# akanazawa/human_dynamics

Hardware: AMD Instinct MI355X
Metric: frames/sec/GPU (ResNet+temporal+SMPL, 224x224); SMPL verts max-abs-err (higher is better)
Workload: dtype f16x3

## Files before the change

human_dynamics_amd/csrc/stem.hip:

```cpp
#include <type_traits>
#include <utility>

#include "common.h"
#include "hmmr_hip.h"

namespace {
constexpr int IMG = 224, CONV = 112, POOL = 56, CO = 64;
constexpr int PT = 8;
constexpr int CT = 2 * PT + 1;
constexpr int IP = 2 * CT + 5;
constexpr int IPW = 40;
constexpr int NPIX = CT * CT;
constexpr int MT = (NPIX + 31) / 32;
constexpr int TAPK = 32;
constexpr int WK = 256;

template <typename T> struct StemLds {
    static constexpr int PXB = 4 * (int)sizeof(T);
    static constexpr int PATCH = IP * IPW * PXB;
    static constexpr int WROW = 7 * TAPK * (int)sizeof(T) + 16;
    static constexpr int WTS = CO * WROW;
    static constexpr int CST = MT * 32 * CO * (int)sizeof(T);
    static constexpr int TOTAL = PATCH + (WTS > CST ? WTS : CST);
};

template <typename T> struct StemFrag;
template <> struct StemFrag<float> { typedef f32x4 type; };
template <> struct StemFrag<bf16_t> { typedef bf16x8 type; };

__device__ __forceinline__ f32x16 stem_mma(const f32x4& a, const f32x4& b, f32x16 c) {
#pragma unroll
    for (int j = 0; j < 4; ++j) c = __builtin_amdgcn_mfma_f32_32x32x2f32(a[j], b[j], c, 0, 0, 0);
    return c;
}
__device__ __forceinline__ f32x16 stem_mma(const bf16x8& a, const bf16x8& b, f32x16 c) {
    return __builtin_amdgcn_mfma_f32_32x32x16_bf16(a, b, c, 0, 0, 0);
}

__device__ __forceinline__ void store_rgbx(float* o, float r, float g, float b) {
    *(f32x4*)o = f32x4{r, g, b, 0.f};
}
__device__ __forceinline__ void store_rgbx(bf16_t* o, float r, float g, float b) {
    typedef __attribute__((ext_vector_type(4))) __bf16 bf16x4;
    *(bf16x4*)o = bf16x4{(bf16_t)r, (bf16_t)g, (bf16_t)b, (bf16_t)0.f};
}

template <typename T>
__global__ __launch_bounds__(256) void stem_fused_kernel(const float* __restrict__ img, const T* __restrict__ wts,
                                                         const float* __restrict__ bias,
                                                         const float* __restrict__ pscale,
                                                         const float* __restrict__ pshift, T* __restrict__ out,
                                                         int n_real, const T* __restrict__ w1,
                                                         const float* __restrict__ s1, const float* __restrict__ b1,
                                                         T* __restrict__ out_h1) {
    typedef StemLds<T> LD;
    typedef typename StemFrag<T>::type frag_t;
    constexpr int CPT = (int)sizeof(T);
    extern __shared__ __attribute__((aligned(16))) char smem[];
    char* s_patch = smem;
    char* s_w = smem + LD::PATCH;
    T* s_c = (T*)(smem + LD::PATCH);

    const int tid = threadIdx.x, lane = tid & 63;
    const int wave = __builtin_amdgcn_readfirstlane(tid >> 6);
    const int ty = blockIdx.x / (POOL / PT), tx = blockIdx.x % (POOL / PT);
    const int n = blockIdx.y;
    const int cy0 = 2 * PT * ty, cx0 = 2 * PT * tx;
    const int iy0 = 2 * cy0 - 3, ix0 = 2 * cx0 - 3;

    const float* im = img + (long long)n * IMG * IMG * 3;
    for (int i = tid; i < IP * 11; i += 256) {
        const int py = i / 11, q = i - py * 11;
        const int gy = iy0 + py, gx = ix0 - 1 + 4 * q;
        float f[12];
#pragma unroll
        for (int e = 0; e < 12; ++e) f[e] = 0.f;
        if (n < n_real && (unsigned)gy < (unsigned)IMG && (unsigned)gx < (unsigned)IMG) {
            const f32x4* p = (const f32x4*)(im + (gy * IMG + gx) * 3);
            const f32x4 v0 = p[0], v1 = p[1], v2 = p[2];
#pragma unroll
            for (int e = 0; e < 4; ++e) { f[e] = v0[e]; f[4 + e] = v1[e]; f[8 + e] = v2[e]; }
        }
#pragma unroll
        for (int e = 0; e < 4; ++e) {
            const int px = 4 * q - 1 + e;
            if ((unsigned)px < (unsigned)IPW) {
                T* o = (T*)(s_patch + (py * IPW + px) * LD::PXB);
                store_rgbx(o, f[3 * e], f[3 * e + 1], f[3 * e + 2]);
            }
        }
    }
    constexpr int SLOTS_PER_ROW = 7 * TAPK * (int)sizeof(T) / 16;
    for (int i = tid; i < CO * SLOTS_PER_ROW; i += 256) {
        const int row = i / SLOTS_PER_ROW, sl = i - row * SLOTS_PER_ROW;
        *(u32x4*)(s_w + row * LD::WROW + sl * 16) = *(const u32x4*)((const char*)(wts + (long long)row * WK) + sl * 16);
    }
    __syncthreads();

    const int lr = lane & 31, lh = lane >> 5;
    constexpr int MPW = (MT + 3) / 4;
    f32x16 acc[MPW][2];
#pragma unroll
    for (int i = 0; i < MPW; ++i)
#pragma unroll
        for (int j = 0; j < 2; ++j)
#pragma unroll
            for (int r = 0; r < 16; ++r) acc[i][j][r] = 0.f;
    int abase[MPW];
#pragma unroll
    for (int i = 0; i < MPW; ++i) {
        int p = (wave + 4 * i) * 32 + lr;
        if (p >= NPIX) p = 0;
        const int cy = p / CT, cx = p - cy * CT;
        abase[i] = ((2 * cy) * IPW + 2 * cx) * LD::PXB + lh * 16;
    }
    const int bbase = lr * LD::WROW + lh * 16;
#pragma unroll 1
    for (int ky = 0; ky < 7; ++ky) {
#pragma unroll
        for (int c = 0; c < CPT; ++c) {
            const frag_t b0 = *(const frag_t*)(s_w + bbase + ky * TAPK * (int)sizeof(T) + c * 32);
            const frag_t b1 = *(const frag_t*)(s_w + bbase + 32 * LD::WROW + ky * TAPK * (int)sizeof(T) + c * 32);
#pragma unroll
            for (int i = 0; i < MPW; ++i) {
                if (wave + 4 * i < MT) {
                    const frag_t a = *(const frag_t*)(s_patch + abase[i] + ky * IPW * LD::PXB + c * 32);
                    acc[i][0] = stem_mma(a, b0, acc[i][0]);
                    acc[i][1] = stem_mma(a, b1, acc[i][1]);
                }
            }
        }
    }
    __syncthreads();

#pragma unroll
    for (int i = 0; i < MPW; ++i) {
        if (wave + 4 * i < MT) {
#pragma unroll
            for (int j = 0; j < 2; ++j) {
                const int ch = j * 32 + lr;
                const float bch = bias[ch];
#pragma unroll
                for (int r = 0; r < 16; ++r) {
                    const int p = (wave + 4 * i) * 32 + (r & 3) + 8 * (r >> 2) + 4 * lh;
                    s_c[p * CO + ch] = elem_traits<T>::from_f32(acc[i][j][r] + bch);
                }
            }
        }
    }
    __syncthreads();

    for (int it = tid; it < PT * PT * (CO / 8); it += 256) {
        const int v8 = it & 7, pp = it >> 3;
        const int py = pp / PT, px = pp - py * PT;
        float m[8];
#pragma unroll
        for (int j = 0; j < 8; ++j) m[j] = -3.0e38f;
#pragma unroll
        for (int dy = 0; dy < 3; ++dy) {
            if (cy0 + 2 * py + dy >= CONV) continue;
#pragma unroll
            for (int dx = 0; dx < 3; ++dx) {
                if (cx0 + 2 * px + dx >= CONV) continue;
                float v[8];
                load8(s_c + ((2 * py + dy) * CT + 2 * px + dx) * CO + v8 * 8, v);
#pragma unroll
                for (int j = 0; j < 8; ++j) m[j] = fmaxf(m[j], v[j]);
            }
        }
        float sc[8], sh[8];
        load8(pscale + v8 * 8, sc); load8(pshift + v8 * 8, sh);
#pragma unroll
        for (int j = 0; j < 8; ++j) m[j] = fmaxf(fmaf(m[j], sc[j], sh[j]), 0.f);
        store8(out + (((long long)n * POOL + PT * ty + py) * POOL + PT * tx + px) * CO + v8 * 8, m);
        if constexpr (sizeof(T) == 2) {
            if (out_h1) store8((T*)(s_patch + pp * 128 + ((v8 ^ ((pp >> 1) & 7)) << 4)), m);
        }
    }
    if constexpr (sizeof(T) == 2) {
        if (!out_h1) return;
        __syncthreads();
        const int lr = lane & 31, lh = lane >> 5, fsw = (lr >> 1) & 7;
        const int wn = wave >> 1, wm = wave & 1;
        f32x16 acc1;
#pragma unroll
        for (int r = 0; r < 16; ++r) acc1[r] = 0.f;
#pragma unroll
        for (int kc = 0; kc < 4; ++kc) {
            const bf16x8 a = *(const bf16x8*)(w1 + (long long)(wn * 32 + lr) * 64 + kc * 16 + lh * 8);
            const bf16x8 b = *(const bf16x8*)(s_patch + (wm * 32 + lr) * 128 + (((2 * kc + lh) ^ fsw) << 4));
            acc1 = __builtin_amdgcn_mfma_f32_32x32x16_bf16(a, b, acc1, 0, 0, 0);
        }
        char* s_o = smem + LD::PATCH;
#pragma unroll
        for (int g = 0; g < 4; ++g) {
            const int cl = wn * 32 + 8 * g + 4 * lh;
            const f32x4 s4 = *(const f32x4*)(s1 + cl), b4 = *(const f32x4*)(b1 + cl);
            typedef __attribute__((ext_vector_type(4))) __bf16 bf16x4;
            bf16x4 o;
#pragma unroll
            for (int j = 0; j < 4; ++j) o[j] = (bf16_t)fmaxf(fmaf(acc1[4 * g + j], s4[j], b4[j]), 0.f);
            *(bf16x4*)(s_o + (wm * 32 + lr) * 128 + (((cl >> 3) ^ fsw) << 4) + 8 * lh) = o;
        }
        __syncthreads();
        for (int it = tid; it < PT * PT * (CO / 8); it += 256) {
            const int ps = it & 7, pp = it >> 3, ls = ps ^ ((pp >> 1) & 7);
            const int py = pp / PT, px = pp - py * PT;
            *(u32x4*)(out_h1 + (((long long)n * POOL + PT * ty + py) * POOL + PT * tx + px) * CO + ls * 8) =
                *(const u32x4*)(s_o + pp * 128 + ps * 16);
        }
    }
}
}


namespace {
constexpr int X3_NT = 320, X3_CO = 32;
constexpr int X3_PLANE = IP * IPW * 8;
constexpr int X3_WROW = 7 * TAPK * 2 + 16;
constexpr int X3_WPLANE = X3_CO * X3_WROW;
constexpr int X3_STAGE = MT * 32 * X3_CO * 4;
constexpr int X3_PTILE = PT * PT * 128;
constexpr int X3_LDS0 = 2 * X3_PLANE + (2 * X3_WPLANE > X3_STAGE ? 2 * X3_WPLANE : X3_STAGE);
constexpr int X3_LDS = X3_LDS0 + X3_PTILE;
static_assert(2 * X3_PTILE <= 2 * X3_PLANE + X3_PTILE && 2 * X3_LDS <= 160 * 1024, "two workgroups per CU");

__global__ __launch_bounds__(X3_NT) void stem_fused_split_kernel(const float* __restrict__ img, const bsplit_t* __restrict__ wts,
                                                                 const float* __restrict__ wscale,
                                                                 const float* __restrict__ bias, const float* __restrict__ pscale,
                                                                 const float* __restrict__ pshift, bsplit_t* __restrict__ out,
                                                                 int n_real, const char* __restrict__ w1f, const float* __restrict__ s1,
                                                                 const float* __restrict__ b1, bsplit_t* __restrict__ out_h1) {
    extern __shared__ __attribute__((aligned(16))) char smem[];
    char* s_ph = smem;
    char* s_pl = smem + X3_PLANE;
    char* s_wh = smem + 2 * X3_PLANE;
    char* s_wl = s_wh + X3_WPLANE;
    float* s_c = (float*)(smem + 2 * X3_PLANE);

    const int tid = threadIdx.x, lane = tid & 63;
    const int wave = __builtin_amdgcn_readfirstlane(tid >> 6);
    const int ty = blockIdx.x / (POOL / PT), tx = blockIdx.x % (POOL / PT);
    const int n = blockIdx.y;
    const int cy0 = 2 * PT * ty, cx0 = 2 * PT * tx;
    const int iy0 = 2 * cy0 - 3, ix0 = 2 * cx0 - 3;

    const float* im = img + (long long)n * IMG * IMG * 3;
    float satin = 0.f;
    for (int i = tid; i < IP * 11; i += X3_NT) {
        const int py = i / 11, q = i - py * 11;
        const int gy = iy0 + py, gx = ix0 - 1 + 4 * q;
        float f[12];
#pragma unroll
        for (int e = 0; e < 12; ++e) f[e] = 0.f;
        if (n < n_real && (unsigned)gy < (unsigned)IMG && (unsigned)gx < (unsigned)IMG) {
            const f32x4* p = (const f32x4*)(im + (gy * IMG + gx) * 3);
            const f32x4 v0 = p[0], v1 = p[1], v2 = p[2];
#pragma unroll
            for (int e = 0; e < 4; ++e) { f[e] = v0[e]; f[4 + e] = v1[e]; f[8 + e] = v2[e]; }
#pragma unroll
            for (int e = 0; e < 12; e += 2) satin = sat_acc(satin, f[e], f[e + 1]);
        }
#pragma unroll
        for (int e = 0; e < 4; ++e) {
            const int px = 4 * q - 1 + e;
            if ((unsigned)px < (unsigned)IPW) {
                typedef __attribute__((ext_vector_type(4))) shalf_t shalf4;
                shalf4 h, l;
#pragma unroll
                for (int c = 0; c < 3; ++c) {
                    const float cv = split_clamp(f[3 * e + c]);
                    h[c] = (shalf_t)cv;
                    l[c] = (shalf_t)(cv - (float)h[c]);
                }
                h[3] = (shalf_t)0.f; l[3] = (shalf_t)0.f;
                *(shalf4*)(s_ph + (py * IPW + px) * 8) = h;
                *(shalf4*)(s_pl + (py * IPW + px) * 8) = l;
            }
        }
    }
    split_flag_max(satin);
#pragma unroll 1
    for (int ch0 = 0; ch0 < CO; ch0 += X3_CO) {
    if (ch0) __syncthreads();
    for (int i = tid; i < X3_CO * 28; i += X3_NT) {
        const int row = i / 28, g = i - row * 28;
        const u32x4* src = (const u32x4*)((const char*)wts + (long long)(ch0 + row) * (WK * 4) + g * 32);
        *(u32x4*)(s_wh + row * X3_WROW + g * 16) = src[0];
        *(u32x4*)(s_wl + row * X3_WROW + g * 16) = src[1];
    }
    __syncthreads();

    const int lr = lane & 31, lh = lane >> 5;
    constexpr int MPW = MT / 5;
    static_assert(MPW * 5 == MT, "10 row tiles over 5 waves");
    f32x16 acc[MPW];
#pragma unroll
    for (int i = 0; i < MPW; ++i)
#pragma unroll
        for (int r = 0; r < 16; ++r) acc[i][r] = 0.f;
    int abase[MPW];
#pragma unroll
    for (int i = 0; i < MPW; ++i) {
        int p = (wave + 5 * i) * 32 + lr;
        if (p >= NPIX) p = 0;
        const int cy = p / CT, cx = p - cy * CT;
        abase[i] = ((2 * cy) * IPW + 2 * cx) * 8 + lh * 16;
    }
    const int bbase = lr * X3_WROW + lh * 16;
    const unsigned lds0 = (unsigned)(unsigned long long)(__attribute__((address_space(3))) void*)smem;
    const unsigned aw = lds0 + 2 * X3_PLANE + bbase;
    unsigned ap[MPW];
#pragma unroll
    for (int i = 0; i < MPW; ++i) ap[i] = lds0 + abase[i];
    shalf8 fb[2][2], fa[2][MPW][2];
#define STEM_RD(dst, addr, OFF) asm volatile("ds_read_b128 %0, %1 offset:%2" : "=v"(dst) : "v"(addr), "n"(OFF))
    auto load_step = [&](auto s_c, int set) {
        constexpr int S = decltype(s_c)::value, KY = S >> 1, C = S & 1;
        shalf8& bh = fb[set][0];
        shalf8& bl = fb[set][1];
        STEM_RD(bh, aw, KY * 64 + C * 32);
        STEM_RD(bl, aw, X3_WPLANE + KY * 64 + C * 32);
#pragma unroll
        for (int i = 0; i < MPW; ++i) {
            shalf8& ah = fa[set][i][0];
            shalf8& al = fa[set][i][1];
            const unsigned ad = ap[i];
            STEM_RD(ah, ad, KY * IPW * 8 + C * 32);
            STEM_RD(al, ad, X3_PLANE + KY * IPW * 8 + C * 32);
        }
    };
    auto k_step = [&](auto s_c) {
        constexpr int S = decltype(s_c)::value, CUR = S & 1;
        if constexpr (S + 1 < 14) load_step(std::integral_constant<int, (S + 1 < 14 ? S + 1 : 13)>{}, CUR ^ 1);
#pragma unroll
        for (int i = 0; i < MPW; ++i) {
            acc[i] = mfma_split(fa[CUR][i][1], fb[CUR][0], acc[i]);
            acc[i] = mfma_split(fa[CUR][i][0], fb[CUR][1], acc[i]);
            acc[i] = mfma_split(fa[CUR][i][0], fb[CUR][0], acc[i]);
        }
        __builtin_amdgcn_sched_barrier(0);
        __builtin_amdgcn_s_waitcnt(63 | (7 << 4) | (0 << 8) | (3 << 14));
        __builtin_amdgcn_sched_barrier(0);
    };
    load_step(std::integral_constant<int, 0>{}, 0);
    __builtin_amdgcn_s_waitcnt(63 | (7 << 4) | (0 << 8) | (3 << 14));
    __builtin_amdgcn_sched_barrier(0);
    auto k_steps = [&](auto... S) { (k_step(S), ...); };
    k_steps(std::integral_constant<int, 0>{}, std::integral_constant<int, 1>{}, std::integral_constant<int, 2>{}, std::integral_constant<int, 3>{},
            std::integral_constant<int, 4>{}, std::integral_constant<int, 5>{}, std::integral_constant<int, 6>{}, std::integral_constant<int, 7>{},
            std::integral_constant<int, 8>{}, std::integral_constant<int, 9>{}, std::integral_constant<int, 10>{}, std::integral_constant<int, 11>{},
            std::integral_constant<int, 12>{}, std::integral_constant<int, 13>{});
#undef STEM_RD
    __syncthreads();

    {
        const float bch = bias[ch0 + lr];
        const float sch = wscale ? wscale[ch0 + lr] : 1.0f;
#pragma unroll
        for (int i = 0; i < MPW; ++i)
#pragma unroll
            for (int r = 0; r < 16; ++r) {
                const int p = (wave + 5 * i) * 32 + (r & 3) + 8 * (r >> 2) + 4 * lh;
                s_c[p * X3_CO + lr] = stored_value<bsplit_t>(fmaf(acc[i][r], sch, bch));
            }
    }
    __syncthreads();

    for (int it = tid; it < PT * PT * (X3_CO / 8); it += X3_NT) {
        const int v8 = it & 3, pp = it >> 2;
        const int py = pp / PT, px = pp - py * PT;
        float m[8];
#pragma unroll
        for (int j = 0; j < 8; ++j) m[j] = -3.0e38f;
#pragma unroll
        for (int dy = 0; dy < 3; ++dy) {
            if (cy0 + 2 * py + dy >= CONV) continue;
#pragma unroll
            for (int dx = 0; dx < 3; ++dx) {
                if (cx0 + 2 * px + dx >= CONV) continue;
                float v[8];
                load8(s_c + ((2 * py + dy) * CT + 2 * px + dx) * X3_CO + v8 * 8, v);
#pragma unroll
                for (int j = 0; j < 8; ++j) m[j] = fmaxf(m[j], v[j]);
            }
        }
        float sc[8], sh[8];
        load8(pscale + ch0 + v8 * 8, sc); load8(pshift + ch0 + v8 * 8, sh);
#pragma unroll
        for (int j = 0; j < 8; ++j) m[j] = fmaxf(fmaf(m[j], sc[j], sh[j]), 0.f);
        bsplit_t* o = out + (((long long)n * POOL + PT * ty + py) * POOL + PT * tx + px) * CO + ch0 + v8 * 8;
        store8(o, m);
        if (w1f) {
            shalf8 hi, lo;
#pragma unroll
            for (int j = 0; j < 8; ++j) {
                const float cv = split_clamp(m[j]);
                hi[j] = (shalf_t)cv;
                lo[j] = (shalf_t)(cv - (float)hi[j]);
            }
            char* pt = (ch0 ? smem : smem + X3_LDS0) + pp * 128 + ((v8 ^ (pp & 3)) << 5);
            *(shalf8*)pt = hi;
            *(shalf8*)(pt + 16) = lo;
        }
    }
    }
    if (!w1f) return;
    __syncthreads();
    if (wave < 4) {
        const int lr = lane & 31, lh = lane >> 5;
        const int wn = wave >> 1, wm = wave & 1;
        const int p = wm * 32 + lr;
        f32x16 acc1;
#pragma unroll
        for (int r = 0; r < 16; ++r) acc1[r] = 0.f;
#pragma unroll
        for (int kc = 0; kc < 4; ++kc) {
            const shalf8* wp = (const shalf8*)(w1f + ((long long)((wn * 4 + kc) * 64 + lane)) * 32);
            wfrag wf; wf.hi = wp[0]; wf.lo = wp[1];
            const int g = (2 * kc + lh) & 3;
            const char* pt = (kc >= 2 ? smem : smem + X3_LDS0) + p * 128 + ((g ^ (p & 3)) << 5);
            acc1 = mma3(wf, *(const shalf8*)pt, *(const shalf8*)(pt + 16), acc1);
        }
        const int py = p >> 3, px = p & 7;
        bsplit_t* o = out_h1 + (((long long)n * POOL + PT * ty + py) * POOL + PT * tx + px) * CO;
        float satmax = 0.f;
#pragma unroll
        for (int g = 0; g < 4; ++g) {
            const int ch = wn * 32 + 8 * g + 4 * lh;
            const f32x4 s4 = *(const f32x4*)(s1 + ch), b4 = *(const f32x4*)(b1 + ch);
            float v[4];
#pragma unroll
            for (int e = 0; e < 4; ++e) v[e] = fmaf(acc1[4 * g + e], s4[e], b4[e]);
            unsigned h2[2], l2[2];
            split4_mix(v, 0.f, h2, l2, satmax);
            char* og = (char*)o + (wn * 4 + g) * 32 + 8 * lh;
            *(unsigned long long*)og = (unsigned long long)h2[0] | ((unsigned long long)h2[1] << 32);
            *(unsigned long long*)(og + 16) = (unsigned long long)l2[0] | ((unsigned long long)l2[1] << 32);
        }
        split_flag_max(satmax);
    }
}
}

int hmmr_stem_fused(const float* images, int n_real, int n, const void* wts, const float* wscale, const float* bias,
                    const float* pscale, const float* pshift, void* out, int dtype, hipStream_t s,
                    const void* w1, const float* s1, const float* b1, void* out_h1) {
    if (dtype == HMMR_F16X3) {
        auto kern = stem_fused_split_kernel;
        static DeviceOnce oncex3;
        if (const unsigned long long bit = oncex3.due()) {
            HMMR_CHECK_HIP(hipFuncSetAttribute((const void*)kern, hipFuncAttributeMaxDynamicSharedMemorySize, X3_LDS));
            oncex3.mark(bit);
        }
        hipLaunchKernelGGL(kern, dim3((POOL / PT) * (POOL / PT), n), dim3(X3_NT), X3_LDS, s, images,
                           (const bsplit_t*)wts, wscale, bias, pscale, pshift, (bsplit_t*)out, n_real, (const char*)w1, s1, b1,
                           (bsplit_t*)out_h1);
    } else if (dtype == HMMR_BF16) {
        auto kern = stem_fused_kernel<bf16_t>;
        static DeviceOnce once16;
        if (const unsigned long long bit = once16.due()) {
            HMMR_CHECK_HIP(hipFuncSetAttribute((const void*)kern, hipFuncAttributeMaxDynamicSharedMemorySize, StemLds<bf16_t>::TOTAL));
            once16.mark(bit);
        }
        hipLaunchKernelGGL(kern, dim3((POOL / PT) * (POOL / PT), n), dim3(256), StemLds<bf16_t>::TOTAL, s, images,
                           (const bf16_t*)wts, bias, pscale, pshift, (bf16_t*)out, n_real, (const bf16_t*)w1, s1, b1,
                           (bf16_t*)out_h1);
    } else {
        auto kern = stem_fused_kernel<float>;
        static DeviceOnce once32;
        if (const unsigned long long bit = once32.due()) {
            HMMR_CHECK_HIP(hipFuncSetAttribute((const void*)kern, hipFuncAttributeMaxDynamicSharedMemorySize, StemLds<float>::TOTAL));
            once32.mark(bit);
        }
        hipLaunchKernelGGL(kern, dim3((POOL / PT) * (POOL / PT), n), dim3(256), StemLds<float>::TOTAL, s, images,
                           (const float*)wts, bias, pscale, pshift, (float*)out, n_real, (const float*)nullptr,
                           (const float*)nullptr, (const float*)nullptr, (float*)nullptr);
    }
    HMMR_CHECK_HIP(hipGetLastError());
    return 0;
}
```

human_dynamics_amd/devflags.py:

```python
from __future__ import annotations

import os

FLAGS = {
    "LIB_PATH": ("", "load this shared object instead of human_dynamics_amd/libhmmr_hip.so (tools/probe_build.sh)"),
    "STEM": ("", "u[nfused] | f[used]: hmmr_debug_t.stem_route"),
    "STEM_C1": ("1", "0: hmmr_debug_t.stem_no_conv1"),
    "GEMM_PROBE": ("0", "hmmr_debug_t.gemm_probe (only the -DHMMR_GEMM_PROBE development build reads the field; results are garbage there)"),
    "RESNET_CHUNK": ("", "encode the batch in sequential chunks of this many frames (heuristic tiles)"),
    "FUSE_PREACT": ("block1,block2,block3,block4", "blocks whose units pre-activate inside the operand staging of conv1 / shortcut"),
    "FUSE_TAIL": ("1", "0 | 1 | block1 | noconv2 | conv2b1 | nosc | nostride2: which fused bottleneck tails the packer marks"),
    "FUSE_SC": ("1", "0 | 1 | all: shortcut + conv1 as one column-split GEMM (1: blocks 3-4)"),
    "PREACT_FIRST": ("0", "1: a block's first unit fuses its pre-activation too"),
    "FOLD_SC": ("", "0 | 1: conv shortcut folded into conv3's K (default: f16x3 only)"),
    "PATCH_3X3": ("2", "the stride-1 3x3 layers of blocks 2-4 (f16x3): 2 = the one-wave-per-SIMD stream kernel (k_order 2), 1 = the 8-wave patch kernels (k_order 1), 0 = tap-major K order and the im2col gather; the three differ by fp32 accumulation rounding"),
    "B1_STREAM": ("0", "1: the conv2 of block1/unit_1 and unit_2 as a launch of the 3x3 stream kernel (64-channel tiles) instead of inside their fused tails (f16x3; measured equal)"),
    "B1_UNIT": ("1", "0: block1/unit_1 and unit_2 as the round-3 LDS-panel tails with conv2 inside (tap-major conv2) instead of the whole-unit kernel of csrc/b1_unit.hip (f16x3; conv2 chunk-major: the two differ by fp32 accumulation rounding)"),
    "STREAM_1X1": ("1", "0: the conv1 of block 4 and of block2/unit_1 and block3/unit_1's shortcut + conv1 as launches of the 8-wave tiles (csrc/gemm_conv.hip) instead of the two-ring stream kernel of csrc/conv1x1_stream.hip (f16x3; the two differ by fp32 accumulation rounding)"),
    "UNIT_PAIR": ("1", "0 | 1 | block2 | block3: the stride-1 units of blocks 2-3 as register-resident unit pairs (csrc/unit_pair.hip; f16x3)"),
    "AUTOTUNE": ("1", "0: no per-layer tile tuning pass (shipped table / library heuristic only)"),
    "TILE_TABLE": ("1", "0: ignore the shipped tile tables (tile_tables.json), tune or fall back to the heuristic"),
    "TILE_CACHE": ("", "json file the tuned tile tables are read from / written to (profiling runs)"),
    "TUNE_TILES": ("5,6,3,1,2,7,8,11,4", "hmmr_conv_desc_t.tile candidates of the tuner"),
    "RESNET_STREAMS": ("2", "contiguous parts a large batch is encoded as, on concurrent streams"),
    "RESNET_PRIORITY": ("-1", "HIP priority of the ResNet side streams"),
    "TAIL_PRIORITY": ("0", "HIP priority of the tail stream (dist.ShardedPredictor)"),
    "STEP_BUFFERS": ("2", "calls in flight of a pipelined ShardedPredictor (record buffers, and encode streams with STEP_STREAMS): 2, or more to try"),
    "STEP_STREAMS": ("1", "0: keep consecutive steps' ResNet passes on one stream (dist.ShardedPredictor)"),
    "STREAM_POISON": ("", "1: evaluation/streaming.py fills a chunk's record buffer with NaN before its tail writes it (a row nobody wrote, or a download that ran early, shows on the host)"),
    "STREAM_TRACE": ("", "1: evaluation/streaming.py prints the host and device timeline of a call"),
}


def get(name):
    default = FLAGS[name][0]
    return os.environ.get("HMMR_" + name, default)


def is_set(name):
    return ("HMMR_" + name) in os.environ and name in FLAGS
```

human_dynamics_amd/engine.py:

```python
from __future__ import annotations

import ctypes as C
import os
import threading
import time

import numpy as np
import torch

from . import _lib as L
from . import assets, devflags, packing

DTYPES = {"f32": L.HMMR_F32, "fp32": L.HMMR_F32, "float32": L.HMMR_F32,
          "bf16": L.HMMR_BF16, "bfloat16": L.HMMR_BF16,
          "f16x3": L.HMMR_F16X3, "split": L.HMMR_F16X3}
DTYPE_NAMES = {L.HMMR_F32: "f32", L.HMMR_BF16: "bf16", L.HMMR_F16X3: "f16x3"}
DEFAULT_DTYPE = "f16x3"
TILE_TABLES = os.path.join(os.path.dirname(os.path.abspath(__file__)), "tile_tables.json")


def set_debug(stem_route=0, stem_no_conv1=0, gemm_probe=0, smpl_blend_mfma=0, ief_no_group=0, pair_min_pixels=0, pair_two_tile_min=0, pair_form=0):
    d = L.Debug()
    d.stem_route, d.stem_no_conv1, d.gemm_probe = int(stem_route), int(stem_no_conv1), int(gemm_probe)
    d.smpl_blend_mfma, d.ief_no_group, d.pair_min_pixels = int(smpl_blend_mfma), int(ief_no_group), int(pair_min_pixels)
    d.pair_two_tile_min, d.pair_form = int(pair_two_tile_min), int(pair_form)
    L.load().hmmr_set_debug(C.byref(d))


def _debug_from_env():
    e = devflags.get("STEM")
    c1 = devflags.get("STEM_C1")
    probe = int(devflags.get("GEMM_PROBE") or 0)
    if e or c1 == "0" or probe or _debug_from_env.was_set:
        set_debug(stem_route={"u": 1, "f": 2}.get(e[:1], 0), stem_no_conv1=int(c1 == "0"), gemm_probe=probe)
        _debug_from_env.was_set = bool(e or c1 == "0" or probe)


_debug_from_env.was_set = False


def _dt(d):
    if isinstance(d, str):
        if d == "bf16x3":
            import warnings
            warnings.warn("dtype 'bf16x3' is now 'f16x3' (split operands with fp16 halves since round 3)", DeprecationWarning, stacklevel=3)
            d = "f16x3"
        if d not in DTYPES:
            raise ValueError("unknown operand mode %r: use one of %s" % (d, ", ".join(sorted(set(DTYPES)))))
        return DTYPES[d]
    return int(d)


def _packer_choices(fold_sc=None, fuse_tail=None, patch_3x3=None, unit_pair=None, b1_stream=None, b1_unit=None, stem_conv1=True,
                    stream_1x1=None):
    def _flag_choice(name):
        v = devflags.get(name)
        return {"0": False, "1": True}.get(v, v)

    def pick(arg, flag):
        return flag if arg is None else arg
    fsc, fold = _flag_choice("FUSE_SC"), _flag_choice("FOLD_SC")
    return dict(fuse_preact_blocks=tuple(b for b in devflags.get("FUSE_PREACT").split(",") if b),
                fuse_tail=pick(fuse_tail, _flag_choice("FUSE_TAIL")),
                fuse_sc=fsc if isinstance(fsc, bool) else "all",
                fuse_preact_first=_flag_choice("PREACT_FIRST") is not False,
                fold_sc=pick(fold_sc, fold if isinstance(fold, bool) else None),
                patch_3x3=pick(patch_3x3, int(devflags.get("PATCH_3X3"))),
                unit_pair=pick(unit_pair, _flag_choice("UNIT_PAIR")),
                b1_stream=pick(b1_stream, _flag_choice("B1_STREAM") is True),
                b1_unit=pick(b1_unit, _flag_choice("B1_UNIT") is True),
                stem_conv1=stem_conv1,
                stream_1x1=pick(stream_1x1, _flag_choice("STREAM_1X1") is True))


class _Workspace(object):

    def __init__(self, device):
        self.device, self.buf = device, None

    def get(self, nbytes):
        if self.buf is None or self.buf.numel() < nbytes:
            self.buf = torch.empty(int(nbytes), dtype=torch.uint8, device=self.device)
        return self.buf


class HmmrEngine(object):

    def __init__(self, weights, smpl, dtype=DEFAULT_DTYPE, device="cuda:0", num_conv_layers=3,
                 delta_t_values=(-5, 5), joint_type="cocoplus", resnet_chunk=0,
                 temporal_dtype=None, ief_dtype=None, autotune=True, fold_sc=None, fuse_tail=None, patch_3x3=None,
                 unit_pair=None, b1_stream=None, b1_unit=None, stem_conv1=True, stream_1x1=None):
        self.lib = L.load()
        _debug_from_env()
        if not torch.cuda.is_available():
            raise L.HmmrError("HmmrEngine needs a HIP device (torch.cuda.is_available() is False)")
        self.device = torch.device(device)
        torch.cuda.set_device(self.device)
        self.dtype = _dt(dtype)
        self.temporal_dtype = self.dtype if temporal_dtype is None else _dt(temporal_dtype)
        self.ief_dtype = self.dtype if ief_dtype is None else _dt(ief_dtype)
        self.resnet_chunk = int(devflags.get("RESNET_CHUNK") or resnet_chunk)
        self.store = packing.DeviceStore(self.device)
        self.num_conv_layers = num_conv_layers
        self.delta_keys = sorted(int(d) for d in delta_t_values)
        w = weights if weights is not None else {}
        for name, v in w.items():
            a_ = np.asarray(v)
            if a_.dtype.kind == "f" and not np.isfinite(a_).all():
                raise ValueError("variable %r holds %d non-finite value(s)" % (name, int((~np.isfinite(a_)).sum())))
        choices = _packer_choices(fold_sc=fold_sc, fuse_tail=fuse_tail, patch_3x3=patch_3x3, unit_pair=unit_pair, b1_stream=b1_stream,
                                  b1_unit=b1_unit, stem_conv1=stem_conv1, stream_1x1=stream_1x1)
        self.rw = packing.pack_resnet(w, self.dtype, self.store, **choices) if "resnet_v2_50/conv1/weights" in w else None
        self.tw = (packing.pack_temporal(w, self.temporal_dtype, self.store, num_conv_layers)
                   if assets.temporal_scopes(0)[1] + "/weights" in w else None)
        self.hw = packing.pack_hallucinator(w, self.temporal_dtype, self.store)
        if "single_view_ief/3D_module/fc1/weights" in w and "mean_param" in w:
            self.iw, self.reg_keys = packing.pack_ief(w, self.ief_dtype, self.store, self.delta_keys)
        else:
            self.iw, self.reg_keys = None, [0]
        all_f32 = (self.dtype, self.temporal_dtype, self.ief_dtype) == (L.HMMR_F32,) * 3
        self.sc = packing.pack_smpl(smpl, self.store, joint_type, split=not all_f32) if smpl is not None else None
        self.num_kps = self.sc.num_kps if self.sc is not None else assets.NUM_KPS
        self.num_verts = self.sc.num_verts if self.sc is not None else assets.NUM_VERTS
        self._ws = {k: _Workspace(self.device) for k in ("resnet", "temporal", "ief", "smpl", "hal")}
        at = devflags.get("AUTOTUNE")
        self.autotune = False if (not autotune or at == "0") else ("force" if (autotune == "force" or at == "force") else True)
        self._tiles, self._shipped = {}, set()
        self.tune_log = []
        self._tile_cache = devflags.get("TILE_CACHE")
        sources = []
        if self.autotune != "force" and devflags.get("TILE_TABLE") != "0" and os.path.exists(TILE_TABLES):
            sources.append((TILE_TABLES, True))
        if self._tile_cache and os.path.exists(self._tile_cache):
            sources.append((self._tile_cache, False))
        for path, shipped in sources:
            import json
            for key, tab in json.load(open(path)).items():
                if key.startswith("_"):
                    continue
                dt, nt = key.split(":")
                if int(dt) == self.dtype:
                    self._tiles[int(nt)] = {(int(k.split(":")[0]), k.split(":")[1]): int(v) for k, v in tab.items()}
                    if shipped:
                        self._shipped.add(int(nt))
        self.resnet_streams = int(devflags.get("RESNET_STREAMS"))
        self._side_streams = []

    @staticmethod
    def _need(packed, names):
        if packed is None:
            raise L.HmmrError("the loaded weights have no %s variables: this stage was not packed" % names)

    def _stream(self):
        return torch.cuda.current_stream(self.device).cuda_stream

    _carried_flags = {}

    def run_flags(self, clear=False):
        key = (self.device.type, self.device.index)
        v = self._device_flags(clear) | HmmrEngine._carried_flags.get(key, 0)
        if clear:
            HmmrEngine._carried_flags.pop(key, None)
        return v

    def _device_flags(self, clear):
        torch.cuda.synchronize(self.device)
        with torch.cuda.device(self.device):
            v = C.c_uint(0)
            L.check(self.lib.hmmr_run_flags(C.byref(v), int(bool(clear))), "hmmr_run_flags")
        return int(v.value)

    def flag_scope(self):
        return _FlagScope(self)

    def to_device(self, a, dtype=torch.float32):
        if isinstance(a, torch.Tensor):
            return a.to(self.device, dtype).contiguous()
        return torch.from_numpy(np.ascontiguousarray(a)).to(self.device).to(dtype).contiguous()

    _TUNE_TILES = tuple(int(t) for t in devflags.get("TUNE_TILES").split(","))
    _TUNE_MIN_FRAMES = 32
    _SPLIT_MIN_FRAMES = 176

    def _resnet_layers(self):
        out, slot = [], 3
        for u in range(L.RESNET_UNITS):
            names = (["shortcut"] if self.rw.unit[u].shortcut.w else []) + ["conv1", "conv2", "conv3"]
            for nm in names:
                out.append((slot, u, nm))
                slot += 1
        return out

    def _layer_of(self, u, nm):
        U = self.rw.unit[u]
        if nm == "conv3" and U.c3sc.w:
            return U.c3sc
        return getattr(U, nm)

    @staticmethod
    def _tile_for(lay, cand, cout, dtype=None, nm="conv2"):
        if lay.k_order == 2 and nm != "conv2":
            t = {5: 22, 6: 23, 3: 24, 1: 25, 2: 26, 4: 29}.get(cand, cand if (22 <= cand <= 26 or cand == 29) else 0)
            return 0 if (nm == "conv3" and t in (22, 23, 29)) else t
        if lay.k_order == 2:
            if cout == 64:
                return {5: 19, 6: 20}.get(cand, cand if cand in (19, 20) else 0)
            t = {5: 13, 6: 14, 3: 15, 1: 16, 2: 17, 7: 18, 8: 12, 11: 21, 4: 27, 9: 28}.get(cand, cand if (12 <= cand <= 18 or cand in (21, 27, 28)) else 0)
            return 0 if (t in (21, 27, 28) and dtype == L.HMMR_BF16) else t
        if lay.k_order:
            cand = {7: 9, 8: 10}.get(cand, cand)
            if cand == 11 and dtype == L.HMMR_BF16:
                return 0
            return cand if (cand in (9, 11) and cout % 128 == 0) or (cand == 10 and cout % 256 == 0) else 0
        if cand not in (1, 2, 3, 5, 6, 7, 8) or (cand in (1, 5, 7) and cout % 128) or (cand == 8 and cout % 256):
            return 0
        return cand

    def _layer_cout(self, u, nm):
        U = self.rw.unit[u]
        if nm == "shortcut" and U.sc_c1.w:
            return U.depth + U.base
        return U.base if nm in ("conv1", "conv2") else U.depth

    def _set_tiles(self, table):
        for (u, nm), t in table.items():
            self._layer_of(u, nm).tile = self._tile_for(self._layer_of(u, nm), int(t), self._layer_cout(u, nm), self.dtype, nm)

    def _needs_tuning(self, nt):
        if not self.autotune or nt < self._TUNE_MIN_FRAMES or nt in self._tiles or torch.cuda.is_current_stream_capturing():
            return False
        if len(self.tune_log) >= 8:
            return False
        if self.autotune == "force":
            return True
        return not any(max(k, nt) <= 1.3 * min(k, nt) for k in self._tiles)

    def _tune_resnet(self, images, n, n_zero, ws_key="resnet", reps=3):
        layers = self._resnet_layers()
        t_start = time.perf_counter()
        nt = n + n_zero
        nbytes = self.lib.hmmr_resnet50_workspace_bytes(nt, self.dtype)
        ws = self._ws.setdefault(ws_key, _Workspace(self.device)).get(nbytes)
        phi = torch.empty((nt, 2048), dtype=torch.float32, device=self.device)
        src = images.data_ptr() if n else None
        best = {}
        for cand in (0,) + self._TUNE_TILES:
            for slot, u, nm in layers:
                lay = self._layer_of(u, nm)
                lay.tile = self._tile_for(lay, cand, self._layer_cout(u, nm), self.dtype, nm)
            t = None
            for rep in range(reps):
                pm = (C.c_float * L.RESNET_PROF_SLOTS)()
                L.check(self.lib.hmmr_resnet50_fwd(C.byref(self.rw), src, n, n_zero, phi.data_ptr(), ws.data_ptr(),
                                                   nbytes, self._stream(), pm), "hmmr_resnet50_fwd")
                cur = np.frombuffer(pm, dtype=np.float32).copy()
                t = cur if (t is None or rep == 0) else np.minimum(t, cur)
            for slot, u, nm in layers:
                tile = self._layer_of(u, nm).tile
                if (u, nm) not in best or t[slot] < best[(u, nm)][0] * 0.98:
                    best[(u, nm)] = (float(t[slot]), tile)
        table = {k: v[1] for k, v in best.items()}
        self.tune_log.append((nt, round((time.perf_counter() - t_start) * 1e3, 1)))
        if self._tile_cache:
            import json
            old = json.load(open(self._tile_cache)) if os.path.exists(self._tile_cache) else {}
            old["%d:%d" % (self.dtype, nt)] = {"%d:%s" % k: v for k, v in table.items()}
            json.dump(old, open(self._tile_cache, "w"))
        return table

    def _resnet_pass(self, images, n, n_zero, phi, ws_key, prof=False, tune=True):
        nt = n + n_zero
        table = None
        if tune and nt >= self._TUNE_MIN_FRAMES:
            if self._needs_tuning(nt):
                self._tiles[nt] = self._tune_resnet(images, n, n_zero, ws_key)
            if self._tiles:
                table = self._tiles[min(self._tiles, key=lambda k: abs(k - nt))]
        if table is not None:
            self._set_tiles(table)
        elif self._tiles:
            self._set_tiles({k: 0 for k in next(iter(self._tiles.values()))})
        nbytes = self.lib.hmmr_resnet50_workspace_bytes(nt, self.dtype)
        ws = self._ws.setdefault(ws_key, _Workspace(self.device)).get(nbytes)
        pm = (C.c_float * L.RESNET_PROF_SLOTS)() if prof else None
        L.check(self.lib.hmmr_resnet50_fwd(C.byref(self.rw), images.data_ptr() if n else None, n, n_zero,
                                           phi.data_ptr(), ws.data_ptr(), nbytes, self._stream(), pm),
                "hmmr_resnet50_fwd")
        return np.frombuffer(pm, dtype=np.float32).astype(np.float64) if prof else None

    def resnet_cuts(self, n, parts=None):
        parts = self.resnet_streams if parts is None else int(parts)
        if parts < 2 or n < self._SPLIT_MIN_FRAMES or self.resnet_chunk > 0:
            return [0, n]
        return [(i * n) // parts for i in range(parts + 1)]

    def resnet(self, images, prof=False, n_zero=0, out=None, ws_key="resnet", parts=None):
        self._need(self.rw, "resnet_v2_50/*")
        images = self.to_device(images)
        n = images.shape[0]
        assert n == 0 or tuple(images.shape[1:]) == (224, 224, 3), images.shape
        nt = n + n_zero
        if out is not None:
            assert out.is_cuda and out.dtype == torch.float32 and out.shape == (nt, 2048) and out.is_contiguous()
        phi = out if out is not None else torch.empty((nt, 2048), dtype=torch.float32, device=self.device)
        if self.resnet_chunk > 0:
            chunk, i = self.resnet_chunk, 0
            prof_tot = np.zeros(L.RESNET_PROF_SLOTS, np.float64) if prof else None
            while i < nt:
                c_real = max(0, min(chunk, n - i))
                c_zero = min(chunk - c_real, nt - i - c_real) if i + c_real >= n else 0
                pm = self._resnet_pass(images[i:i + c_real], c_real, c_zero, phi[i:i + c_real + c_zero], "resnet",
                                       prof, tune=False)
                if prof:
                    prof_tot += pm
                i += c_real + c_zero
            return (phi, prof_tot) if prof else phi
        parts = self.resnet_streams if parts is None else int(parts)
        if prof or parts < 2 or n < self._SPLIT_MIN_FRAMES or torch.cuda.is_current_stream_capturing():
            pm = self._resnet_pass(images, n, n_zero, phi, ws_key, prof)
            return (phi, pm) if prof else phi
        cur = torch.cuda.current_stream(self.device)
        self.side_stream(parts - 1)
        cuts = [(i * n) // parts for i in range(parts + 1)]
        if self.autotune:
            for i in range(parts):
                ni, nz = cuts[i + 1] - cuts[i], (n_zero if i == parts - 1 else 0)
                if self._needs_tuning(ni + nz):
                    self._tiles[ni + nz] = self._tune_resnet(images[cuts[i]:cuts[i + 1]], ni, nz, "resnet%d" % i)
        for i in range(parts):
            side = self._side_streams[i]
            side.wait_stream(cur)
            with torch.cuda.stream(side):
                nz = n_zero if i == parts - 1 else 0
                self._resnet_pass(images[cuts[i]:cuts[i + 1]], cuts[i + 1] - cuts[i], nz,
                                  phi[cuts[i]:cuts[i + 1] + nz], "resnet%d" % i)
        for i in range(parts):
            cur.wait_stream(self._side_streams[i])
# ... 461 lines not shown
```

Baseline: 39620.

## Add persistent stem kernel with resident weights and prefetched next-tile patches

Adds a persistent f16x3 stem kernel, launched with one 640-thread workgroup per CU, that loops over tiles. The conv weights, per-channel constants and conv1 weight fragments are loaded once per workgroup. The next tile's image patch is fetched into registers while the current tile's MFMA conv, maxpool and conv1 run. This replaces the per-tile kernel as the default route; the old kernel stays reachable through a debug flag. It aims to remove repeated weight loads and launch-per-tile overhead and to hide global load latency. In exchange it loses the two-workgroups-per-CU occupancy and adds compile-time timing-probe macros.

```diff
diff --git a/human_dynamics_amd/csrc/stem.hip b/human_dynamics_amd/csrc/stem.hip
--- a/human_dynamics_amd/csrc/stem.hip
+++ b/human_dynamics_amd/csrc/stem.hip
@@ -214,6 +214,31 @@
 }
 
 
+#ifndef STEM_PROBE_BITS
+#define STEM_PROBE_BITS 0
+#endif
+#define XP_DROP(bit) ((STEM_PROBE_BITS & (bit)) != 0)
+#ifdef STEM_PROBE
+__device__ unsigned long long g_stem_probe[8];
+extern "C" int hmmr_stem_probe(unsigned long long* out, int clear) {
+    if (hipDeviceSynchronize() != hipSuccess || hipMemcpyFromSymbol(out, HIP_SYMBOL(g_stem_probe), sizeof(g_stem_probe)) != hipSuccess) return -2;
+    if (clear) {
+        const unsigned long long z[8] = {};
+        if (hipMemcpyToSymbol(HIP_SYMBOL(g_stem_probe), z, sizeof(z)) != hipSuccess) return -2;
+    }
+    return 0;
+}
+#define STEM_PROBE_BEGIN(W) const bool probe_on = wave == (W); unsigned long long probe_acc[8] = {}, probe_t = __builtin_amdgcn_s_memtime()
+#define STEM_STAMP(slot) do { if (probe_on) { const unsigned long long now_ = __builtin_amdgcn_s_memtime(); probe_acc[slot] += now_ - probe_t; probe_t = now_; } } while (0)
+#define STEM_PROBE_TILE() do { probe_acc[5] += 1; } while (0)
+#define STEM_PROBE_END() do { if (probe_on && lane == 0) { for (int i_ = 0; i_ < 8; ++i_) atomicAdd(&g_stem_probe[i_], probe_acc[i_]); } } while (0)
+#else
+#define STEM_PROBE_BEGIN(W) do {} while (0)
+#define STEM_STAMP(slot) do {} while (0)
+#define STEM_PROBE_TILE() do {} while (0)
+#define STEM_PROBE_END() do {} while (0)
+#endif
+
 namespace {
 constexpr int X3_NT = 320, X3_CO = 32;
 constexpr int X3_PLANE = IP * IPW * 8;
@@ -245,6 +270,8 @@
     const int cy0 = 2 * PT * ty, cx0 = 2 * PT * tx;
     const int iy0 = 2 * cy0 - 3, ix0 = 2 * cx0 - 3;
 
+    STEM_PROBE_BEGIN(0);
+    STEM_PROBE_TILE();
     const float* im = img + (long long)n * IMG * IMG * 3;
     float satin = 0.f;
     for (int i = tid; i < IP * 11; i += X3_NT) {
@@ -283,6 +310,7 @@
 #pragma unroll 1
     for (int ch0 = 0; ch0 < CO; ch0 += X3_CO) {
     if (ch0) __syncthreads();
+    STEM_STAMP(ch0 ? 3 : 0);
     for (int i = tid; i < X3_CO * 28; i += X3_NT) {
         const int row = i / 28, g = i - row * 28;
         const u32x4* src = (const u32x4*)((const char*)wts + (long long)(ch0 + row) * (WK * 4) + g * 32);
@@ -290,6 +318,7 @@
         *(u32x4*)(s_wl + row * X3_WROW + g * 16) = src[1];
     }
     __syncthreads();
+    STEM_STAMP(1);
 
     const int lr = lane & 31, lh = lane >> 5;
     constexpr int MPW = MT / 5;
@@ -366,6 +395,7 @@
             }
     }
     __syncthreads();
+    STEM_STAMP(2);
 
     for (int it = tid; it < PT * PT * (X3_CO / 8); it += X3_NT) {
         const int v8 = it & 3, pp = it >> 2;
@@ -405,8 +435,12 @@
         }
     }
     }
+#ifdef STEM_PROBE
+    if (!w1f) { STEM_STAMP(3); STEM_PROBE_END(); }
+#endif
     if (!w1f) return;
     __syncthreads();
+    STEM_STAMP(3);
     if (wave < 4) {
         const int lr = lane & 31, lh = lane >> 5;
         const int wn = wave >> 1, wm = wave & 1;
@@ -440,13 +474,276 @@
         }
         split_flag_max(satmax);
     }
+    STEM_STAMP(4);
+    STEM_PROBE_END();
+}
+__device__ __forceinline__ void lds_barrier() { asm volatile("s_waitcnt lgkmcnt(0)\n\ts_barrier" ::: "memory"); }
+constexpr int XP_NT = 640;
+constexpr int XP_W = 0;
+constexpr int XP_P = XP_W + 4 * X3_WPLANE;
+constexpr int XP_CROW = 40;
+constexpr int XP_C = XP_P + 2 * X3_PLANE;
+constexpr int XP_T = XP_C + MT * 32 * XP_CROW * 4;
+constexpr int XP_K = XP_T + 2 * X3_PTILE;
+constexpr int XP_LDS = XP_K + 6 * CO * 4;
+constexpr int XP_ITEMS = IP * 11;
+static_assert(XP_LDS <= 160 * 1024 && XP_ITEMS <= XP_NT && XP_P % 16 == 0 && XP_C % 16 == 0 && XP_T % 16 == 0 && XP_K % 16 == 0, "one workgroup per CU");
+
+__global__ __launch_bounds__(XP_NT) void stem_persistent_split_kernel(const float* __restrict__ img, const bsplit_t* __restrict__ wts,
+                                                                      const float* __restrict__ wscale,
+                                                                      const float* __restrict__ bias, const float* __restrict__ pscale,
+                                                                      const float* __restrict__ pshift, bsplit_t* __restrict__ out,
+                                                                      int n_real, const char* __restrict__ w1f, const float* __restrict__ s1,
+                                                                      const float* __restrict__ b1, bsplit_t* __restrict__ out_h1, int n_tiles) {
+    extern __shared__ __attribute__((aligned(16))) char smem[];
+    char* s_ph = smem + XP_P;
+    char* s_pl = s_ph + X3_PLANE;
+    float* s_c = (float*)(smem + XP_C);
+    float* s_k = (float*)(smem + XP_K);
+
+    const int tid = threadIdx.x, lane = tid & 63;
+    const int wave = __builtin_amdgcn_readfirstlane(tid >> 6);
+    const int lr = lane & 31, lh = lane >> 5;
+    const int G = gridDim.x;
+    const int L = xcd_remap(blockIdx.x, G);
+    STEM_PROBE_BEGIN(2);
+
+    for (int i = tid; i < CO * 28; i += XP_NT) {
+        const int row = i / 28, g = i - row * 28;
+        const u32x4* src = (const u32x4*)((const char*)wts + (long long)row * (WK * 4) + g * 32);
+        char* dst = smem + XP_W + (row >> 5) * (2 * X3_WPLANE) + (row & 31) * X3_WROW + g * 16;
+        *(u32x4*)dst = src[0];
+        *(u32x4*)(dst + X3_WPLANE) = src[1];
+    }
+    if (tid < CO) {
+        s_k[tid] = bias[tid];
+        s_k[CO + tid] = wscale ? wscale[tid] : 1.0f;
+        s_k[2 * CO + tid] = pscale[tid];
+        s_k[3 * CO + tid] = pshift[tid];
+        s_k[4 * CO + tid] = w1f ? s1[tid] : 0.f;
+        s_k[5 * CO + tid] = w1f ? b1[tid] : 0.f;
+    }
+    const bool c1_wave = w1f && (wave & 2) && wave < 8;
+    const int c1_id = ((wave >> 2) << 1) | (wave & 1);
+    const int wn = (c1_id >> 1) & 1, wm = c1_id & 1;
+    wfrag wf[4] = {};
+    if (c1_wave) {
+#pragma unroll
+        for (int kc = 0; kc < 4; ++kc) {
+            const shalf8* wp = (const shalf8*)(w1f + ((long long)((wn * 4 + kc) * 64 + lane)) * 32);
+            wf[kc].hi = wp[0]; wf[kc].lo = wp[1];
+        }
+    }
+
+    const int item = XP_NT - 1 - tid;
+    const int ppy = item / 11, pq = item - ppy * 11;
+    float satin = 0.f;
+    auto patch_request = [&](int t, float (&f)[12], bool on) {
+#pragma unroll
+        for (int e = 0; e < 12; ++e) f[e] = 0.f;
+        if (!on || item >= XP_ITEMS) return;
+        const int n = t / 49, r = t - n * 49, ty = r / 7, tx = r - ty * 7;
+        const int gy = 4 * PT * ty - 3 + ppy, gx = 4 * PT * tx - 4 + 4 * pq;
+        if (!XP_DROP(8) && n < n_real && (unsigned)gy < (unsigned)IMG && (unsigned)gx < (unsigned)IMG) {
+            const f32x4* p = (const f32x4*)(img + (long long)n * IMG * IMG * 3 + (gy * IMG + gx) * 3);
+            const f32x4 v0 = p[0], v1 = p[1], v2 = p[2];
+#pragma unroll
+            for (int e = 0; e < 4; ++e) { f[e] = v0[e]; f[4 + e] = v1[e]; f[8 + e] = v2[e]; }
+        }
+    };
+    auto patch_store = [&](const float (&f)[12]) {
+        if (item >= XP_ITEMS) return;
+#pragma unroll
+        for (int e = 0; e < 12; e += 2) satin = sat_acc(satin, f[e], f[e + 1]);
+#pragma unroll
+        for (int e = 0; e < 4; ++e) {
+            const int px = 4 * pq - 1 + e;
+            if ((unsigned)px < (unsigned)IPW) {
+                typedef __attribute__((ext_vector_type(4))) shalf_t shalf4;
+                shalf4 h, l;
+#pragma unroll
+                for (int c = 0; c < 3; ++c) {
+                    const float cv = split_clamp(f[3 * e + c]);
+                    h[c] = (shalf_t)cv;
+                    l[c] = (shalf_t)(cv - (float)h[c]);
+                }
+                h[3] = (shalf_t)0.f; l[3] = (shalf_t)0.f;
+                *(shalf4*)(s_ph + (ppy * IPW + px) * 8) = h;
+                *(shalf4*)(s_pl + (ppy * IPW + px) * 8) = l;
+            }
+        }
+    };
+    {
+        float f[12];
+        patch_request(L, f, L < n_tiles);
+        patch_store(f);
+    }
+    __syncthreads();
+    STEM_STAMP(6);
+
+    int p0 = wave * 32 + lr;
+    if (p0 >= NPIX) p0 = 0;
+    const unsigned lds0 = (unsigned)(unsigned long long)(__attribute__((address_space(3))) void*)smem;
+    const unsigned ap = lds0 + XP_P + ((2 * (p0 / CT)) * IPW + 2 * (p0 % CT)) * 8 + lh * 16;
+    const unsigned aw0 = lds0 + XP_W + lr * X3_WROW + lh * 16;
+    float satmax1 = 0.f;
+
+#pragma unroll 1
+    for (int t = L; t < n_tiles; t += G) {
+        STEM_PROBE_TILE();
+        const int n = t / 49, rt = t - n * 49, ty = rt / 7, tx = rt - ty * 7;
+        const int cy0 = 2 * PT * ty, cx0 = 2 * PT * tx;
+        const bool more = t + G < n_tiles;
+        float f[12];
+        patch_request(t + G, f, more);
+        STEM_STAMP(0);
+#pragma unroll
+        for (int ch0 = 0; ch0 < CO; ch0 += X3_CO) {
+            f32x16 acc;
+#pragma unroll
+            for (int r = 0; r < 16; ++r) acc[r] = 0.f;
+            const unsigned adr[2] = {aw0 + (ch0 ? 2 * X3_WPLANE : 0), ap};
+            shalf8 fb[2][2], fa[2][2];
+#define STEM_RD(dst, addr, OFF) asm volatile("ds_read_b128 %0, %1 offset:%2" : "=v"(dst) : "v"(addr), "n"(OFF))
+            auto load_step = [&](auto s_c, int set) {
+                constexpr int S = decltype(s_c)::value, KY = S >> 1, C = S & 1;
+                const unsigned aw = adr[0], ad = adr[1];
+                shalf8& bh = fb[set][0];
+                shalf8& bl = fb[set][1];
+                shalf8& ah = fa[set][0];
+                shalf8& al = fa[set][1];
+                STEM_RD(bh, aw, KY * 64 + C * 32);
+                STEM_RD(bl, aw, X3_WPLANE + KY * 64 + C * 32);
+                STEM_RD(ah, ad, KY * IPW * 8 + C * 32);
+                STEM_RD(al, ad, X3_PLANE + KY * IPW * 8 + C * 32);
+            };
+            auto k_step = [&](auto s_c) {
+                constexpr int S = decltype(s_c)::value, CUR = S & 1;
+                if constexpr (S + 1 < 14) load_step(std::integral_constant<int, (S + 1 < 14 ? S + 1 : 13)>{}, CUR ^ 1);
+                acc = mfma_split(fa[CUR][1], fb[CUR][0], acc);
+                acc = mfma_split(fa[CUR][0], fb[CUR][1], acc);
+                acc = mfma_split(fa[CUR][0], fb[CUR][0], acc);
+                __builtin_amdgcn_sched_barrier(0);
+                __builtin_amdgcn_s_waitcnt(63 | (7 << 4) | (0 << 8) | (3 << 14));
+                __builtin_amdgcn_sched_barrier(0);
+            };
+            load_step(std::integral_constant<int, 0>{}, 0);
+            __builtin_amdgcn_s_waitcnt(63 | (7 << 4) | (0 << 8) | (3 << 14));
+            __builtin_amdgcn_sched_barrier(0);
+            auto k_steps = [&](auto... S) { (k_step(S), ...); };
+            if (!XP_DROP(4))
+            k_steps(std::integral_constant<int, 0>{}, std::integral_constant<int, 1>{}, std::integral_constant<int, 2>{}, std::integral_constant<int, 3>{},
+                    std::integral_constant<int, 4>{}, std::integral_constant<int, 5>{}, std::integral_constant<int, 6>{}, std::integral_constant<int, 7>{},
+                    std::integral_constant<int, 8>{}, std::integral_constant<int, 9>{}, std::integral_constant<int, 10>{}, std::integral_constant<int, 11>{},
+                    std::integral_constant<int, 12>{}, std::integral_constant<int, 13>{});
+#undef STEM_RD
+            {
+                const float bch = s_k[ch0 + lr], sch = s_k[CO + ch0 + lr];
+#pragma unroll
+                for (int r = 0; r < 16; ++r) {
+                    const int p = wave * 32 + (r & 3) + 8 * (r >> 2) + 4 * lh;
+                    s_c[p * XP_CROW + lr] = stored_value<bsplit_t>(fmaf(acc[r], sch, bch));
+                }
+            }
+            lds_barrier();
+            STEM_STAMP(2);
+
+            if (ch0) {
+#pragma unroll
+                for (int e = 0; e < 12; ++e) asm volatile("" : "+v"(f[e]));
+                if (more) patch_store(f);
+            }
+            if (!XP_DROP(16) && tid < PT * PT * (X3_CO / 8)) {
+                const int v8 = tid & 3, pp = tid >> 2;
+                const int py = pp / PT, px = pp - py * PT;
+                float m[8];
+#pragma unroll
+                for (int j = 0; j < 8; ++j) m[j] = -3.0e38f;
+#pragma unroll
+                for (int dy = 0; dy < 3; ++dy) {
+                    if (cy0 + 2 * py + dy >= CONV) continue;
+#pragma unroll
+                    for (int dx = 0; dx < 3; ++dx) {
+                        if (cx0 + 2 * px + dx >= CONV) continue;
+                        float v[8];
+                        load8(s_c + ((2 * py + dy) * CT + 2 * px + dx) * XP_CROW + v8 * 8, v);
+#pragma unroll
+                        for (int j = 0; j < 8; ++j) m[j] = fmaxf(m[j], v[j]);
+                    }
+                }
+                float sc[8], sh[8];
+                load8(s_k + 2 * CO + ch0 + v8 * 8, sc); load8(s_k + 3 * CO + ch0 + v8 * 8, sh);
+#pragma unroll
+                for (int j = 0; j < 8; ++j) m[j] = fmaxf(fmaf(m[j], sc[j], sh[j]), 0.f);
+                bsplit_t* o = out + (((long long)n * POOL + PT * ty + py) * POOL + PT * tx + px) * CO + ch0 + v8 * 8;
+                if (!XP_DROP(1)) store8(o, m);
+                if (w1f) {
+                    shalf8 hi, lo;
+#pragma unroll
+                    for (int j = 0; j < 8; ++j) {
+                        const float cv = split_clamp(m[j]);
+                        hi[j] = (shalf_t)cv;
+                        lo[j] = (shalf_t)(cv - (float)hi[j]);
+                    }
+                    char* pt = smem + XP_T + (ch0 ? X3_PTILE : 0) + pp * 128 + ((v8 ^ (pp & 3)) << 5);
+                    *(shalf8*)pt = hi;
+                    *(shalf8*)(pt + 16) = lo;
+                }
+            }
+            lds_barrier();
+            STEM_STAMP(3);
+        }
+        if (!XP_DROP(32) && c1_wave) {
+            const int p = wm * 32 + lr;
+            f32x16 acc1;
+#pragma unroll
+            for (int r = 0; r < 16; ++r) acc1[r] = 0.f;
+#pragma unroll
+            for (int kc = 0; kc < 4; ++kc) {
+                const int g = (2 * kc + lh) & 3;
+                const char* pt = smem + XP_T + (kc >= 2 ? X3_PTILE : 0) + p * 128 + ((g ^ (p & 3)) << 5);
+                acc1 = mma3(wf[kc], *(const shalf8*)pt, *(const shalf8*)(pt + 16), acc1);
+            }
+            const int py = p >> 3, px = p & 7;
+            bsplit_t* o = out_h1 + (((long long)n * POOL + PT * ty + py) * POOL + PT * tx + px) * CO;
+#pragma unroll
+            for (int g = 0; g < 4; ++g) {
+                const int ch = wn * 32 + 8 * g + 4 * lh;
+                const f32x4 s4 = *(const f32x4*)(s_k + 4 * CO + ch), b4 = *(const f32x4*)(s_k + 5 * CO + ch);
+                float v[4];
+#pragma unroll
+                for (int e = 0; e < 4; ++e) v[e] = fmaf(acc1[4 * g + e], s4[e], b4[e]);
+                unsigned h2[2], l2[2];
+                split4_mix(v, 0.f, h2, l2, satmax1);
+                char* og = (char*)o + (wn * 4 + g) * 32 + 8 * lh;
+                if (XP_DROP(2)) continue;
+                *(unsigned long long*)og = (unsigned long long)h2[0] | ((unsigned long long)h2[1] << 32);
+                *(unsigned long long*)(og + 16) = (unsigned long long)l2[0] | ((unsigned long long)l2[1] << 32);
+            }
+            STEM_STAMP(4);
+        }
+    }
+    split_flag_max(satin);
+    split_flag_max(satmax1);
+    STEM_PROBE_END();
 }
 }
 
 int hmmr_stem_fused(const float* images, int n_real, int n, const void* wts, const float* wscale, const float* bias,
                     const float* pscale, const float* pshift, void* out, int dtype, hipStream_t s,
                     const void* w1, const float* s1, const float* b1, void* out_h1) {
-    if (dtype == HMMR_F16X3) {
+    if (dtype == HMMR_F16X3 && hmmr_debug_state()->stem_route != 3) {
+        auto kern = stem_persistent_split_kernel;
+        static DeviceOnce oncexp;
+        if (const unsigned long long bit = oncexp.due()) {
+            HMMR_CHECK_HIP(hipFuncSetAttribute((const void*)kern, hipFuncAttributeMaxDynamicSharedMemorySize, XP_LDS));
+            oncexp.mark(bit);
+        }
+        const int tiles = (POOL / PT) * (POOL / PT) * n, cus = hmmr_cu_count(s);
+        HMMR_REQUIRE(n > 0 && n <= 0x7fffffff / 49, "hmmr_stem_fused: bad image count %d", n);
+        hipLaunchKernelGGL(kern, dim3(cus < tiles ? cus : tiles), dim3(XP_NT), XP_LDS, s, images, (const bsplit_t*)wts, wscale, bias, pscale,
+                           pshift, (bsplit_t*)out, n_real, (const char*)w1, s1, b1, (bsplit_t*)out_h1, tiles);
+    } else if (dtype == HMMR_F16X3) {
         auto kern = stem_fused_split_kernel;
         static DeviceOnce oncex3;
         if (const unsigned long long bit = oncex3.due()) {
diff --git a/human_dynamics_amd/devflags.py b/human_dynamics_amd/devflags.py
--- a/human_dynamics_amd/devflags.py
+++ b/human_dynamics_amd/devflags.py
@@ -4,7 +4,7 @@
 
 FLAGS = {
     "LIB_PATH": ("", "load this shared object instead of human_dynamics_amd/libhmmr_hip.so (tools/probe_build.sh)"),
-    "STEM": ("", "u[nfused] | f[used]: hmmr_debug_t.stem_route"),
+    "STEM": ("", "u[nfused] | f[used] | t[ile: the per-tile fused kernel]: hmmr_debug_t.stem_route"),
     "STEM_C1": ("1", "0: hmmr_debug_t.stem_no_conv1"),
     "GEMM_PROBE": ("0", "hmmr_debug_t.gemm_probe (only the -DHMMR_GEMM_PROBE development build reads the field; results are garbage there)"),
     "RESNET_CHUNK": ("", "encode the batch in sequential chunks of this many frames (heuristic tiles)"),
diff --git a/human_dynamics_amd/engine.py b/human_dynamics_amd/engine.py
--- a/human_dynamics_amd/engine.py
+++ b/human_dynamics_amd/engine.py
@@ -32,7 +32,7 @@
     c1 = devflags.get("STEM_C1")
     probe = int(devflags.get("GEMM_PROBE") or 0)
     if e or c1 == "0" or probe or _debug_from_env.was_set:
-        set_debug(stem_route={"u": 1, "f": 2}.get(e[:1], 0), stem_no_conv1=int(c1 == "0"), gemm_probe=probe)
+        set_debug(stem_route={"u": 1, "f": 2, "t": 3}.get(e[:1], 0), stem_no_conv1=int(c1 == "0"), gemm_probe=probe)
         _debug_from_env.was_set = bool(e or c1 == "0" or probe)
 
 
```

Result: no change. 39880 (median of 6 runs) (+0.7%).
